# Jittor/InstanceSegmentation-jittor

Measured on AMD Instinct MI355X. Metric: images/sec (Yolact R50-FPN 550x550, bs=8 per GPU, fp32), higher is better.
Workload: dtype f32; 1 GPU; Yolact R50-FPN 550x550 bs=8/GPU random weights: uint8 upload + FastBaseTransform on the device + backbone+FPN+protonet+heads+Detect(fast-NMS)+550x550 mask assembly (BASELINE configs[1]); global_batch=8, parallelism=batch-sharded x1, RCCL all-gather of detections

## Files before the change

### instancesegmentation-jittor_amd/csrc/engine.h

```cpp
#pragma once
#include "rpn_levels.h"
#include <stdarg.h>

#include <functional>
#include <map>
#include <string>
#include <vector>

#include "../../include/isegmi.h"
#include "common.h"

#define TRY(x)               \
    do {                     \
        int _rc = (x);       \
        if (_rc) return _rc; \
    } while (0)

namespace isegmi {

struct Tensor {
    float* d = nullptr;
    int N = 0, H = 0, W = 0, C = 0;
    int dt = 0;
    int64_t numel() const { return (int64_t)N * H * W * C; }
};

struct ConvLayer {
    int Cout = 0, R = 0, S = 0, Cin = 0;
    float* d_w = nullptr;
    bool f16 = false;
    float* d_scale = nullptr;
    float* d_shift = nullptr;
};

struct RawBuf {
    void* d = nullptr;
    int64_t bytes = 0;
    std::vector<int64_t> shape;
    int dtype = 0;
};

struct StageTime {
    std::string name;
    hipEvent_t ev;
};

constexpr float STEP_OVERLAP_DEFAULT = 1.0f;

struct Engine {
    int kind = 0;
    int max_batch = 0, H = 0, W = 0;
    int cur_H = 0, cur_W = 0;
    int anchor_H = -1, anchor_W = -1;
    hipStream_t stream = nullptr;
    hipStream_t side[3] = {nullptr, nullptr, nullptr};
    hipStream_t cur = nullptr;
    hipStream_t tail = nullptr;
    hipEvent_t tail_done = nullptr;
    bool tail_pending = false;
    hipStream_t heads = nullptr;
    hipStream_t hside[3] = {nullptr, nullptr, nullptr};
    hipEvent_t lat_done[2] = {nullptr, nullptr};
    bool lat_pending[2] = {false, false};
    hipEvent_t heads_done = nullptr;
    bool heads_pending = false;
    bool multi_stream = true;
    hipStream_t lane_stream[2] = {nullptr, nullptr};
    hipStream_t lane_side[2][3] = {{nullptr, nullptr, nullptr}, {nullptr, nullptr, nullptr}};
    int lane_state = 0;
    int lane = 0;
    int lane_next = 0;
    int last_lanes = 1;
    bool lane1_busy = false;
    int64_t lane1_forwards = 0;
    std::string lane_tag;
    bool capturing = false;
    std::map<std::string, hipGraphExec_t> graphs;
    std::map<std::string, int> graph_warm;
    int64_t graph_captures = 0, graph_replays = 0, graph_failures = 0;
    hipStream_t copy = nullptr;
    hipEvent_t in_done[2] = {nullptr, nullptr};
    bool in_pending[2] = {false, false};
    struct Upload { const char* dst = nullptr; int64_t bytes = 0; hipEvent_t done = nullptr; unsigned waited = ~0u; };
    unsigned lane_mask() const { return lane_state == 1 ? 3u : 1u; }
    bool consumed(const Upload& u) const { return (u.waited & lane_mask()) == lane_mask(); }
    std::vector<Upload> uploads;
    std::vector<hipEvent_t> step_marks;
    char* pin_ring = nullptr;
    static constexpr int PIN_SLOTS = 32, PIN_SLOT_BYTES = 4096;
    hipEvent_t pin_ev[PIN_SLOTS] = {};
    bool pin_used[PIN_SLOTS] = {};
    int pin_next = 0;
    int hw_slot = 0;
    void* stream_set = nullptr;
    hipEvent_t dl_done[2] = {nullptr, nullptr};
    bool dl_used[2] = {false, false};
    bool fp16 = false;
    std::vector<hipEvent_t> ev_pool;
    size_t ev_next = 0;
    std::map<std::string, ConvLayer> convs;
    std::map<std::string, RawBuf> tensors;
    std::map<std::string, RawBuf> bufs;
    std::map<std::string, float> params;
    bool finalized = false;
    std::vector<int32_t> last_hw;
    const void* last_hw_ptr = nullptr;
    std::vector<float> last_ratios;
    const void* last_ratios_ptr = nullptr;
    int last_N = 0;
    bool timing = false;
    std::vector<StageTime> marks;
    std::vector<std::pair<std::string, float>> last_times;
    bool conv_timing = false;
    std::vector<std::pair<hipEvent_t, hipEvent_t>> conv_evs;
    std::vector<std::pair<std::string, double>> conv_ev_info;
    bool conv_trace = false;
    std::map<std::string, std::pair<double, double>> conv_layers;
    double conv_flops_pending = 0, conv_flops = 0, conv_ms = 0;
    int64_t conv_launches = 0;
    bool op_timing = false;
    struct OpEv { hipEvent_t a, b; const char* label; double bytes; };
    std::vector<OpEv> op_evs;
    struct OpStat { double us = 0, bytes = 0; int64_t launches = 0; };
    std::map<std::string, OpStat> op_stats;

    float param(const std::string& k, float def) const {
        auto it = params.find(k);
        return it == params.end() ? def : it->second;
    }
};

int eng_buf(Engine& e, const std::string& name, int64_t bytes, void** out, int dtype = 0,
            std::vector<int64_t> shape = {});
int eng_act(Engine& e, const std::string& name, int N, int H, int W, int C, Tensor* t, int dt = 0);
int eng_conv(Engine& e, const std::string& layer, const Tensor& in, int stride, int pad, int act, const Tensor* residual,
             const std::string& out_name, Tensor* out, bool out_f32 = false, bool may_split = false);
int eng_graph_run(Engine& e, const std::string& key, const std::function<int()>& body);
void eng_graph_reset(Engine& e);
int eng_tail_end(Engine& e);
int eng_input_consumed(Engine& e);
int eng_wait_upload(Engine& e, const void* d_ptr, int64_t bytes, hipStream_t st);
int eng_stage_small(Engine& e, const void* h_src, size_t bytes, void* d_dst, hipStream_t st);
hipStream_t eng_results_stream(Engine& e);
int eng_bottleneck_f16(Engine& e, const std::string& block, const Tensor& x, bool first, const std::string& out_name, Tensor* out, bool* fused);
int eng_conv_up2x_f16(Engine& e, const std::string& layer, const Tensor& x, const Tensor& coarse, const std::string& out_name, Tensor* out, bool* merged);
struct ConvGroupItem {
    std::string layer;
    Tensor in;
    int stride = 1, pad = 0, act = 0;
    const Tensor* residual = nullptr;
    std::string out_name;
    Tensor* out = nullptr;
    void* dst = nullptr;
    int out_div = 0;
    int64_t out_img_stride = 0, out_pix_stride = 0;
    bool out_f32 = false;
};
int eng_conv_group(Engine& e, std::vector<ConvGroupItem>& items);
int conv2d_group_launch(int n, const isegmi_conv_desc* const* d, const float* const* in, const float* const* w, const float* const* scale,
                        const float* const* shift, const float* const* res, float* const* out, hipStream_t st);
int eng_rpn_head_f16(Engine& e, const std::string& conv, const std::string& headl, const Tensor& x, const std::string& out_name, Tensor* out, bool* fused);
int eng_stem_pool_f16(Engine& e, const std::string& layer, const Tensor& halo, int H, int W, const std::string& out_name, Tensor* out, bool* fused);
int eng_conv_stem_f16(Engine& e, const std::string& layer, const Tensor& halo, int H, int W, const std::string& out_name, Tensor* out);
int eng_conv_into(Engine& e, const std::string& layer, const Tensor& in, int stride, int pad, int act, void* dst, int out_div,
                  int64_t out_img_stride, int64_t out_pix_stride, bool out_f32 = false);
void eng_mark(Engine& e, const char* name);
int eng_fork(Engine& e, int k);
int eng_join(Engine& e, int k);
struct SideScope {
    Engine& e;
    hipStream_t saved;
    SideScope(Engine& e_, int k) : e(e_), saved(e_.cur) { if (e.multi_stream) e.cur = e.side[k]; }
    ~SideScope() { e.cur = saved; }
};

struct OpScope {
    Engine& e;
    hipStream_t st;
    const char* label;
    double bytes;
    hipEvent_t a = nullptr;
    OpScope(Engine& e_, hipStream_t st_, const char* label_, double bytes_) : e(e_), st(st_), label(label_), bytes(bytes_) {
        if (e.op_timing && !e.capturing && hipEventCreate(&a) == hipSuccess) (void)hipEventRecord(a, st);
    }
    ~OpScope() {
        if (!a) return;
        hipEvent_t b = nullptr;
        if (hipEventCreate(&b) == hipSuccess) { (void)hipEventRecord(b, st); e.op_evs.push_back({a, b, label, bytes}); }
        else (void)hipEventDestroy(a);
    }
};

struct ConvScope {
    Engine& e;
    hipEvent_t a = nullptr, b = nullptr;
    explicit ConvScope(Engine& e_) : e(e_) {
        if (!e.conv_timing) return;
        if (hipEventCreate(&a) == hipSuccess && hipEventCreate(&b) == hipSuccess && hipEventRecord(a, e.cur) == hipSuccess) return;
        drop();
    }
    ~ConvScope() { drop(); }
    void drop() {
        if (a) (void)hipEventDestroy(a);
        if (b) (void)hipEventDestroy(b);
        a = b = nullptr;
    }
    void trace(const std::string& layer, const char* suffix, int N, int H, int W, int Cin, int Cout, int R, int stride, int M, bool res) const {
        if (e.conv_trace) fprintf(stderr, "convlaunch\t%s%s\t%d\t%d\t%d\t%d\t%d\t%d\t%d\t%d\t%d\n", layer.c_str(), suffix, N, H, W, Cin, Cout, R, stride, M, res ? 1 : 0);
    }
    __attribute__((format(printf, 3, 4))) void done(double flops, const char* label_fmt, ...) {
        if (!a) return;
        char label[320];
        va_list ap;
        va_start(ap, label_fmt);
        vsnprintf(label, sizeof(label), label_fmt, ap);
        va_end(ap);
        (void)hipEventRecord(b, e.cur);
        e.conv_evs.push_back({a, b});
        e.conv_ev_info.push_back({label, flops});
        e.conv_flops_pending += flops;
        a = b = nullptr;
    }
};

int resnet_stem(Engine& e, const std::string& layer, const float* d_images, int N, int H, int W, Tensor* pool);
struct ResStage {
    std::string layers;
    std::string bufs;
    int blocks = 0;
    int stride = 1;
    bool stride_in_1x1 = false;
    bool full = false;
    std::string stage;
    bool proj_by_name = false;
    hipEvent_t before_out = nullptr;
};
int resnet_stage(Engine& e, const ResStage& s, const Tensor& in, Tensor* out);
bool eng_has_gn(Engine& e, const std::string& layer);
int eng_gn(Engine& e, const std::string& layer, Tensor* x, const Tensor* residual, bool relu);

int yolact_forward(Engine& e, const float* d_images, int N);
int yolact_postprocess(Engine& e, int h, int w, const int32_t* h_image_hw = nullptr);
int maskrcnn_forward(Engine& e, const float* d_images, int N);
int eng_next_event(Engine& e, hipEvent_t* ev);
int maskrcnn_paste(Engine& e, const float* h_ratios_wh, int out_h, int out_w);

int conv2d_launch(const isegmi_conv_desc* d, const float* in, const float* w, const float* scale, const float* shift,
                  const float* res, float* out, hipStream_t st);
int conv2d_f16_launch(const isegmi_conv_desc* d, const void* in, const void* w, const float* scale, const float* shift, const void* res,
                      void* out, int out_f32, hipStream_t st);
int conv2d_f16_up2x_launch(const isegmi_conv_desc* d, const void* in, const void* w, const float* scale, const float* shift, const void* coarse, int Hc, int Wc,
                           void* out, hipStream_t st);
int conv2d_f16_head_launch(const isegmi_conv_desc* d, const void* in, const void* w, const float* scale, const float* shift, const void* w2,
                           const float* scale2, const float* shift2, int cout2, float* out2, bool* fused, hipStream_t st);
bool stem_pool_f16_supported(int Cout);
int stem_pool_f16_launch(int N, int H, int W, const void* halo, const void* w, const float* scale, const float* shift, void* out, int flags, hipStream_t st);
bool bottleneck_f16_supported(int Cin, int Cmid);
bool bottleneck_f16_ds_supported(int Cin, int Cmid);
int bottleneck_f16_launch(const isegmi_bottleneck_desc* d, const void* x, const void* w1, const float* s1, const float* b1, const void* w2,
                          const float* s2, const float* b2, const void* w3, const float* s3, const float* b3, const void* wd, const float* sd,
                          const float* bd, void* out, hipStream_t st);
int pad_c3_to_f16_halo_launch(const float* in, int N, int H, int W, void* out, hipStream_t st);
int avgpool_full_launch(const float* x, int64_t R, int HW, int C, float* out, hipStream_t st);
int resize_bilinear_f16_launch(const void* in, int N, int H, int W, int C, int Ho, int Wo, const void* add, int relu, void* out, hipStream_t st);
int maxpool_to_f16_launch(const void* in, int in_f16, int N, int H, int W, int C, int k, int s, int p, void* out, hipStream_t st);
int nearest2x_add_f16_launch(const void* coarse, int N, int Hc, int Wc, int C, const void* lat, int H, int W, void* out, hipStream_t st);
int roi_align_f16_launch(const void* const* feats, const int* Hs, const int* Ws, const float* scales, int nlevels, const float* rois,
                         const int* counts, int N, int K, int C, int PH, int PW, int g, int k_min, void* out, hipStream_t st,
                         const int* order = nullptr, const void* tab = nullptr, int aligned = 0);
int roi_prep_launch(const float* rois, const int* counts, int N, int K, const int* Hs, const int* Ws, const float* scales, int nlevels, int k_min, int C,
                    int PH, int PW, int esize, int* order, void* tab, hipStream_t st, int aligned = 0);
int mask_logits_select_f16_launch(const void* feat, int R, int HW, int C, const float* w, const float* b, const int* labels, float* out,
                                  hipStream_t st);
int maxpool_launch(const float* in, int N, int H, int W, int C, int k, int s, int p, float* out, hipStream_t st);
int64_t groupnorm_workspace_bytes(int64_t N, int H, int W, int C, int groups);
bool groupnorm_is_slab(int H, int W);
int groupnorm_launch(const float* x, int64_t N, int H, int W, int C, int groups, const float* gamma, const float* beta, float eps, const float* residual,
                     int relu, float* out, void* ws, int64_t ws_bytes, hipStream_t st);
int resize_bilinear_launch(const float* in, int N, int H, int W, int C, int Ho, int Wo, const float* add, int relu, float* out,
                           hipStream_t st);
int nearest2x_add_launch(const float* coarse, int N, int Hc, int Wc, int C, const float* lat, int H, int W, float* out,
                         hipStream_t st);
int maskiou_conv1_launch(const float* lo, int NK, int PH, int PW, const float* w, const float* b, float* out, hipStream_t st);
int maskiou_rescore_launch(const float* feat, int N, int K, int HW, int C, const int* cls, const float* score, const int* count,
                           float* out, hipStream_t st);
int deform_im2col_launch(const float* x, int N, int H, int W, int C, const float* om, int R, int S, int stride, int pad, int dil,
                         float* out, hipStream_t st);
int pad_c3_c4_launch(const float* in, int64_t npix, float* out, hipStream_t st);
int preprocess_u8_launch(const uint8_t* in, int N, int Hin, int Win, float* out, int Hout, int Wout, int Hpad, int Wpad, int64_t out_img_stride,
                         const float* mean3, const float* std3, int swap_rb, hipStream_t st);
int pad_c3_c32_launch(const float* in, int64_t npix, float* out, hipStream_t st);
int topk_launch(const float* keys, int64_t row_stride, int rows, int n, int k, const int* limit, int rows_per_limit,
                float* out_vals, int* out_idx, int* out_cnt, hipStream_t st);
int yolact_detect_launch(const isegmi_yolact_detect_args* a, hipStream_t st);
int yolact_masks_launch(const float* proto, const float* coeffs, const float* boxes, const int* count, int N, int PH, int PW,
                        int mask_dim, int K, int h, int w, float* ws_lo, uint8_t* out_masks, int64_t* out_boxes, hipStream_t st,
                        const int* image_hw = nullptr, int* win = nullptr, bool clear = true, bool dense_lo = false);

}

struct isegmi_engine {
    isegmi::Engine e;
};
```

### instancesegmentation-jittor_amd/csrc/yolact.cpp

```cpp
#include <string.h>

#include "engine.h"

namespace isegmi {

struct LaneScope {
    Engine& e;
    explicit LaneScope(Engine& e_) : e(e_) { set(e.lane); if (e.lane) e.lane_tag = "@1"; }
    ~LaneScope() { set(0); e.lane_tag.clear(); e.cur = e.stream; }
    void set(int l) {
        if (e.lane_stream[l] == nullptr) return;
        e.stream = e.lane_stream[l];
        for (int k = 0; k < 3; ++k) e.side[k] = e.lane_side[l][k];
    }
};

struct HeadsScope {
    Engine& e;
    hipStream_t s, sd[3];
    bool on = false;
    explicit HeadsScope(Engine& e_) : e(e_), s(e_.stream) { for (int k = 0; k < 3; ++k) sd[k] = e.side[k]; }
    void enter(bool wide) { on = true; e.stream = e.heads; for (int k = 0; k < 3; ++k) e.side[k] = wide ? e.hside[k] : e.heads; e.cur = e.heads; }
    ~HeadsScope() { if (on) { e.stream = s; for (int k = 0; k < 3; ++k) e.side[k] = sd[k]; e.cur = s; } }
};
// ... 141 lines not shown
    if (e.multi_stream && e.tail_pending && !e.capturing) HIP_TRY(hipStreamWaitEvent(e.stream, e.tail_done, 0));
    Tensor proto;
    TRY(eng_fork(e, 0));
    TRY(eng_fork(e, 1));
    TRY(eng_fork(e, 2));
    {
        SideScope sc(e, 0);
        Tensor t, u;
        TRY(eng_conv(e, "proto_net.0", P[0], 1, 1, 1, nullptr, "proto.t0", &t));
        TRY(eng_conv(e, "proto_net.2", t, 1, 1, 1, nullptr, "proto.t1", &u));
        TRY(eng_conv(e, "proto_net.4", u, 1, 1, 1, nullptr, "proto.t2", &t));
        TRY(eng_act(e, "proto.up", N, t.H * 2, t.W * 2, t.C, &u, dt));
        if (dt) TRY(resize_bilinear_f16_launch(t.d, N, t.H, t.W, t.C, t.H * 2, t.W * 2, nullptr, 1, u.d, e.cur));
        else TRY(resize_bilinear_launch(t.d, N, t.H, t.W, t.C, t.H * 2, t.W * 2, nullptr, 1, u.d, e.cur));
        TRY(eng_conv(e, "proto_net.8", u, 1, 1, 1, nullptr, "proto.t3", &t));
        TRY(eng_conv(e, "proto_net.10", t, 1, 0, 1, nullptr, "proto", &proto, true));
    }
    if (grp) {
        Tensor uf[5];
        std::vector<ConvGroupItem> gu(5), gh(5);
        for (int l = 0; l < 5; ++l) {
            gu[l].layer = "prediction_layers.0.upfeature.0"; gu[l].in = P[l]; gu[l].pad = 1; gu[l].act = 1; gu[l].out_name = "head.up" + std::to_string(l); gu[l].out = &uf[l];
        }
        TRY(eng_conv_group(e, gu));
        for (int l = 0; l < 5; ++l) {
            gh[l].layer = "prediction_layers.0.head_cat"; gh[l].in = uf[l]; gh[l].pad = 1; gh[l].act = 0;
            gh[l].dst = (float*)headcat + (int64_t)(off[l] / A) * CH; gh[l].out_div = uf[l].H * uf[l].W;
            gh[l].out_img_stride = (int64_t)(Ptot / A) * CH; gh[l].out_pix_stride = CH; gh[l].out_f32 = true;
        }
        TRY(eng_conv_group(e, gh));
    } else {
        { SideScope sc(e, 1); TRY(head_level(1)); TRY(head_level(3)); }
        { SideScope sc(e, 2); TRY(head_level(2)); TRY(head_level(4)); }
        TRY(head_level(0));
    }
    TRY(eng_join(e, 0));
    TRY(eng_join(e, 1));
    TRY(eng_join(e, 2));
    h->A = A; h->Ptot = Ptot; h->CH = CH; h->fused = fused;
    h->loc = loc; h->conf = conf; h->mask = mask; h->headcat = headcat;
    return ISEGMI_OK;
}

static int detect_args(Engine& e, int N, const HeadOut& h, isegmi_yolact_detect_args* out) {
    const int ncls = kNumClasses, md = kMaskDim, A = h.A, Ptot = h.Ptot;
    const int top_k = (int)e.param("nms_top_k", 200), max_det = (int)e.param("max_num_detections", 100);
    const int nc = ncls - 1;
    isegmi_yolact_detect_args& a = *out;
    memset(&a, 0, sizeof(a));
    a.N = N; a.P = Ptot; a.ncls = ncls; a.mask_dim = md; a.top_k = top_k; a.max_det = max_det;
    a.conf_thresh = e.param("nms_conf_thresh", 0.05f);
    a.nms_thresh = e.param("nms_thresh", 0.5f);
    a.second_threshold = (int)e.param("nms_second_threshold", 0) ? 1 : 0;
    if (h.fused) {
        a.d_conf = a.d_loc = a.d_mask = (const float*)h.headcat;
        a.A = A; a.pix_stride = h.CH; a.off_loc = 0; a.off_conf = A * 4; a.off_mask = A * 4 + A * ncls; a.mask_tanh = 1;
    } else {
        a.d_conf = (const float*)h.conf; a.d_loc = (const float*)h.loc; a.d_mask = (const float*)h.mask;
    }
    a.d_priors = (const float*)e.tensors["priors"].d;
    void* p;
    TRY(eng_buf(e, "ws.scoresT", (int64_t)N * nc * Ptot * 4, &p)); a.d_ws_scoresT = (float*)p;
    TRY(eng_buf(e, "boxes_all", (int64_t)N * Ptot * 16, &p, 0, {N, Ptot, 4})); a.d_ws_boxes = (float*)p;
    TRY(eng_buf(e, "ws.counts", (int64_t)2 * N * 4, &p, 1)); a.d_ws_counts = (int32_t*)p;
    TRY(eng_buf(e, "ws.tk_vals", (int64_t)N * nc * top_k * 4, &p)); a.d_ws_tk_vals = (float*)p;
    TRY(eng_buf(e, "ws.tk_idx", (int64_t)N * nc * top_k * 4, &p, 1)); a.d_ws_tk_idx = (int32_t*)p;
    TRY(eng_buf(e, "ws.tk_cnt", (int64_t)N * nc * 4, &p, 1)); a.d_ws_tk_cnt = (int32_t*)p;
    TRY(eng_buf(e, "ws.cand", (int64_t)N * nc * top_k * 4, &p)); a.d_ws_cand = (float*)p;
    TRY(eng_buf(e, "ws.fin_vals", (int64_t)N * max_det * 4, &p)); a.d_ws_fin_vals = (float*)p;
    TRY(eng_buf(e, "ws.fin_idx", (int64_t)N * max_det * 4, &p, 1)); a.d_ws_fin_idx = (int32_t*)p;
    TRY(eng_buf(e, "ws.fin_cnt", (int64_t)N * 4, &p, 1)); a.d_ws_fin_cnt = (int32_t*)p;
    TRY(eng_buf(e, "det.count", (int64_t)N * 4, &p, 1, {N})); a.d_out_count = (int32_t*)p;
    TRY(eng_buf(e, "det.box", (int64_t)N * max_det * 16, &p, 0, {N, max_det, 4})); a.d_out_boxes = (float*)p;
    TRY(eng_buf(e, "det.score", (int64_t)N * max_det * 4, &p, 0, {N, max_det})); a.d_out_scores = (float*)p;
    TRY(eng_buf(e, "det.class", (int64_t)N * max_det * 4, &p, 1, {N, max_det})); a.d_out_classes = (int32_t*)p;
    TRY(eng_buf(e, "det.coeff", (int64_t)N * max_det * md * 4, &p, 0, {N, max_det, md})); a.d_out_coeffs = (float*)p;
    TRY(eng_buf(e, "det.prior", (int64_t)N * max_det * 4, &p, 1, {N, max_det})); a.d_out_prior = (int32_t*)p;
    return ISEGMI_OK;
}

int yolact_forward(Engine& e, const float* d_images, int N) {
    LaneScope lscope(e);
    e.cur = e.stream;
    const bool pipe = e.multi_stream && !e.capturing && !e.timing && !e.conv_timing && e.heads != nullptr &&
                      e.param("graph", 0.0f) == 0.0f && e.param("pipeline_heads", 1.0f) != 0.0f;
    HeadsScope hscope(e);
    eng_mark(e, "start");
    const int dt = e.fp16 ? 1 : 0;
    if (dt && e.convs.count("prediction_layers.0.head_cat") == 0) { set_error("fp16 Yolact needs the fused prediction head"); return ISEGMI_ERR_STATE; }
    Tensor C[3], P[5];
    if (e.param("darknet", 0.0f) != 0.0f) TRY(darknet_backbone(e, d_images, N, C));
    else TRY(resnet_backbone(e, d_images, N, C));
    if (pipe) {
        hipEvent_t ev;
        TRY(eng_next_event(e, &ev));
        HIP_TRY(hipEventRecord(ev, e.stream));
        HIP_TRY(hipStreamWaitEvent(e.heads, ev, 0));
        const float hs = e.param("heads_side_streams", -1.0f);
        hscope.enter(hs < 0.0f ? N <= 2 : hs != 0.0f);
    } else if (e.heads_pending) {
        HIP_TRY(hipStreamWaitEvent(e.stream, e.heads_done, 0));
        e.heads_pending = false;
    }
    const bool grp = !dt && e.param("conv_groups", 1.0f) != 0.0f && e.param("conv_tile", 0) == 0.0f && e.convs.count("prediction_layers.0.head_cat") != 0;
    TRY(yolact_fpn(e, C, N, grp, pipe, P));
    eng_mark(e, "fpn");
    e.lane_tag.clear();
    HeadOut head;
    TRY(proto_and_heads(e, P, N, grp, &head));
    eng_mark(e, "proto+heads");
    isegmi_yolact_detect_args a;
    TRY(detect_args(e, N, head, &a));
    hipStream_t ds = e.stream;
    if (e.multi_stream) {
        hipEvent_t ev;
        TRY(eng_next_event(e, &ev));
        HIP_TRY(hipEventRecord(ev, e.stream));
        HIP_TRY(hipStreamWaitEvent(e.tail, ev, 0));
        ds = e.tail;
    }
    {
        OpScope op(e, ds, "yolact_detect (softmax + decode + per-class top-k + fast-NMS + gather)",
                   (double)N * a.P * ((double)(4 + a.ncls - 1 + a.mask_dim) * 4) + (double)a.P * 16);
        TRY(yolact_detect_launch(&a, ds));
    }
    if (pipe) { HIP_TRY(hipEventRecord(e.heads_done, e.stream)); e.heads_pending = true; }
    TRY(eng_tail_end(e));
    eng_mark(e, "detect");
    return ISEGMI_OK;
}

int yolact_postprocess(Engine& e, int h, int w, const int32_t* h_image_hw) {
    const int N = e.last_N;
    if (N <= 0) { set_error("postprocess before forward"); return ISEGMI_ERR_STATE; }
    const int K = (int)e.param("max_num_detections", 100);
    RawBuf& proto = e.bufs["proto"];
    const int PH = (int)proto.shape[1], PW = (int)proto.shape[2], md = (int)proto.shape[3];
    void *lo, *masks, *ib;
    hipStream_t rs = (e.multi_stream && e.tail_pending) ? e.tail : e.stream;
    int* d_ihw = nullptr;
    if (h_image_hw) {
        for (int i = 0; i < N; ++i)
            if (h_image_hw[2 * i] <= 0 || h_image_hw[2 * i] > h || h_image_hw[2 * i + 1] <= 0 || h_image_hw[2 * i + 1] > w) { set_error("postprocess: image size outside the plane"); return ISEGMI_ERR_ARG; }
        void* q;
        TRY(eng_buf(e, "pp.image_hw", (int64_t)e.max_batch * 8, &q, 1, {N, 2}));
        d_ihw = (int*)q;
        TRY(eng_stage_small(e, h_image_hw, (size_t)N * 8, d_ihw, rs));
    }
    TRY(eng_buf(e, "ws.lo", (int64_t)N * K * PH * PW * 4, &lo));
    TRY(eng_buf(e, "det.masks", (int64_t)N * K * h * w, &masks, 2, {N, K, h, w}));
    TRY(eng_buf(e, "det.box_int", (int64_t)N * K * 4 * 8, &ib, 3, {N, K, 4}));
    void* wq;
    TRY(eng_buf(e, "det.mask_window", (int64_t)e.max_batch * K * 16, &wq, 1, {N, K, 4}));
    {
        const bool whole = e.param("sparse_masks", 0.0f) == 0.0f;
        OpScope op(e, rs, whole ? "yolact_masks (proto @ coeff -> sigmoid -> crop -> upsample -> threshold, whole uint8 planes)" : "yolact_masks (sparse: box windows only)",
                   (double)N * PH * PW * md * 4 + (double)N * K * md * 4 + (whole ? (double)N * K * h * w : 0.0));
        TRY(yolact_masks_launch((const float*)proto.d, (const float*)e.bufs["det.coeff"].d, (const float*)e.bufs["det.box"].d,
                                (const int*)e.bufs["det.count"].d, N, PH, PW, md, K, h, w, (float*)lo, (uint8_t*)masks, (int64_t*)ib,
                                rs, d_ihw, (int*)wq, whole, e.convs.count("maskiou_net.2") != 0));
    }
    if (e.convs.count("maskiou_net.2")) {
        auto w0 = e.tensors.find("maskiou.w0"), b0 = e.tensors.find("maskiou.b0");
        if (w0 == e.tensors.end() || b0 == e.tensors.end()) { set_error("maskiou_net.0 weights missing"); return ISEGMI_ERR_STATE; }
        hipStream_t saved = e.cur;
        e.cur = rs;
        Tensor t, u;
        TRY(eng_act(e, "maskiou.t0", N * K, (PH - 3) / 2 + 1, (PW - 3) / 2 + 1, 32, &t));
        TRY(maskiou_conv1_launch((const float*)lo, N * K, PH, PW, (const float*)w0->second.d, (const float*)b0->second.d, t.d, rs));
        for (int i = 2; i <= 8; i += 2) {
            if (t.H < 3 || t.W < 3) { e.cur = saved; set_error("input too small for the mask-IoU net (five stride-2 3x3 convs)"); return ISEGMI_ERR_ARG; }
            TRY(eng_conv(e, "maskiou_net." + std::to_string(i), t, 2, 0, 1, nullptr, "maskiou.t" + std::to_string(i), &u));
            t = u;
        }
        TRY(eng_conv(e, "maskiou_net.10", t, 1, 0, 1, nullptr, "maskiou.cls", &u));
        void* ms;
        TRY(eng_buf(e, "det.mask_score", (int64_t)N * K * 4, &ms, 0, {N, K}));
        TRY(maskiou_rescore_launch(u.d, N, K, u.H * u.W, u.C, (const int*)e.bufs["det.class"].d, (const float*)e.bufs["det.score"].d,
                                   (const int*)e.bufs["det.count"].d, (float*)ms, rs));
        e.cur = saved;
    }
    if (rs == e.tail) HIP_TRY(hipEventRecord(e.tail_done, e.tail));
    eng_mark(e, "masks");
    return ISEGMI_OK;
}

}
```

### instancesegmentation-jittor_amd/csrc/yolact_detect.hip

```cpp
#include "../../include/isegmi.h"
#include "common.h"
#include "detmath.h"

namespace isegmi {

constexpr int SM_ROWS = 128;

struct HeadLayout {
    int A;
    int64_t pix_stride;
    int off_loc, off_conf, off_mask, mask_tanh;
};
__device__ __forceinline__ const float* head_ptr(const float* base, const HeadLayout& L, int n, int P, int p, int width, int off) {
    if (L.pix_stride == 0) return base + ((int64_t)n * P + p) * width;
    const int pix = p / L.A, a = p - pix * L.A;
    return base + ((int64_t)n * (P / L.A) + pix) * L.pix_stride + off + a * width;
}

constexpr int SM_PARTS = 4;
__global__ __launch_bounds__(SM_ROWS * SM_PARTS) void yolact_softmax_decode_kernel(
    const float* __restrict__ conf, const float* __restrict__ loc, const float* __restrict__ priors, int P, int C,
    float conf_thresh, const HeadLayout L, float* __restrict__ scoresT, float* __restrict__ boxes, int* __restrict__ keep_count) {
    extern __shared__ float sm[];
    constexpr int NT = SM_ROWS * SM_PARTS;
// ... 38 lines not shown
        if (live) {
            const float s = rsum[t];
            for (int c = part; c < C; c += SM_PARTS) { const float pr = dm_div(r[c], s); r[c] = pr; if (c >= 1) fg = pr > fg ? pr : fg; }
        }
        pmax[part * SM_ROWS + t] = fg;
    }
    __syncthreads();
    float fg = pmax[t];
#pragma unroll
    for (int q = 1; q < SM_PARTS; ++q) { const float v = pmax[q * SM_ROWS + t]; fg = v > fg ? v : fg; }
    const bool kept = live && fg > conf_thresh;
    if (live && part == 1) {
        const float* lp = head_ptr(loc, L, n, P, p, 4, L.off_loc);
        const float4 l = make_float4(lp[0], lp[1], lp[2], lp[3]);
        const float4 q = *(const float4*)(priors + (int64_t)p * 4);
        float tx = l.x * 0.1f; tx = tx * q.z;
        float ty = l.y * 0.1f; ty = ty * q.w;
        const float cx = q.x + tx, cy = q.y + ty;
        const float w = q.z * dm_exp(l.z * 0.2f), h = q.w * dm_exp(l.w * 0.2f);
        const float x1 = cx - dm_div(w, 2.0f), y1 = cy - dm_div(h, 2.0f);
        *(float4*)(boxes + ((int64_t)n * P + p) * 4) = make_float4(x1, y1, w + x1, h + y1);
    }
    const int cnt = __syncthreads_count((kept && part == 0) ? 1 : 0);
    if (threadIdx.x == 0 && cnt) atomicAdd(&keep_count[n], cnt);
    if (live) {
        float* dst = scoresT + (int64_t)n * (C - 1) * P + p;
        for (int c = 1 + part; c < C; c += SM_PARTS) dst[(int64_t)(c - 1) * P] = kept ? r[c] : -1.0f;
    }
}

__device__ __forceinline__ float jaccard(const float4 a, const float4 b) {
    const float mx2 = a.z < b.z ? a.z : b.z, mx1 = a.x > b.x ? a.x : b.x;
    const float my2 = a.w < b.w ? a.w : b.w, my1 = a.y > b.y ? a.y : b.y;
    float iw = mx2 - mx1, ih = my2 - my1;
    iw = iw > 0.0f ? iw : 0.0f;
    ih = ih > 0.0f ? ih : 0.0f;
    const float inter = iw * ih;
    const float aa = (a.z - a.x) * (a.w - a.y), ab = (b.z - b.x) * (b.w - b.y);
    const float uni = aa + ab - inter;
    return dm_div(inter, uni);
}

__global__ __launch_bounds__(1024) void yolact_fast_nms_kernel(const float* __restrict__ boxes, const float* __restrict__ tk_vals,
                                                                const int* __restrict__ tk_idx, const int* __restrict__ tk_cnt,
                                                                int P, int nc, int top_k, float thr, int second_threshold, float conf_thresh,
                                                                float* __restrict__ cand, int* __restrict__ kept_count) {
    __shared__ float4 sb[256];
    __shared__ unsigned char okp[4][256];
    const int c = blockIdx.x, n = blockIdx.y;
    const int base = (n * nc + c) * top_k;
    const int cnt = tk_cnt[n * nc + c];
    const int j = threadIdx.x & 255, part = threadIdx.x >> 8;
    if (part == 0 && j < cnt) sb[j] = *(const float4*)(boxes + ((int64_t)n * P + tk_idx[base + j]) * 4);
    __syncthreads();
    bool ok = true;
    if (j < cnt) {
        const float4 bj = sb[j];
        for (int i = part; i < j; i += 4) {
            const float o = jaccard(sb[i], bj);
            if (!(o <= thr)) { ok = false; break; }
        }
    }
    okp[part][j] = ok ? 1 : 0;
    __syncthreads();
    bool keep = part == 0 && j < cnt && okp[0][j] && okp[1][j] && okp[2][j] && okp[3][j];
    if (second_threshold && keep) keep = tk_vals[base + j] > conf_thresh;
    if (part == 0 && j < top_k) cand[base + j] = keep ? tk_vals[base + j] : -1.0f;
    const int k = __syncthreads_count(keep ? 1 : 0);
    if (threadIdx.x == 0 && k) atomicAdd(&kept_count[n], k);
}

__global__ void yolact_gather_kernel(const float* __restrict__ boxes, const float* __restrict__ mask, const int* __restrict__ tk_idx,
                                     const float* __restrict__ fin_vals, const int* __restrict__ fin_idx,
                                     const int* __restrict__ fin_cnt, int P, int nc, int top_k, int mask_dim, int max_det,
                                     const HeadLayout L,
                                     int* __restrict__ out_count, float* __restrict__ out_boxes, float* __restrict__ out_scores,
                                     int* __restrict__ out_classes, float* __restrict__ out_coeffs, int* __restrict__ out_prior) {
    const int n = blockIdx.x;
    const int cnt = fin_cnt[n];
    if (threadIdx.x == 0) out_count[n] = cnt;
    for (int q = threadIdx.x; q < max_det; q += blockDim.x) {
        const int64_t o = (int64_t)n * max_det + q;
        if (q < cnt) {
            const int flat = fin_idx[o];
            const int c = flat / top_k;
            const int prior = tk_idx[(int64_t)n * nc * top_k + flat];
            *(float4*)(out_boxes + o * 4) = *(const float4*)(boxes + ((int64_t)n * P + prior) * 4);
            out_scores[o] = fin_vals[o];
            out_classes[o] = c;
            out_prior[o] = prior;
            const float* mp = head_ptr(mask, L, n, P, prior, mask_dim, L.off_mask);
            for (int k = 0; k < mask_dim; ++k) out_coeffs[o * mask_dim + k] = L.mask_tanh ? dm_tanh(mp[k]) : mp[k];
        } else {
            *(float4*)(out_boxes + o * 4) = make_float4(0.f, 0.f, 0.f, 0.f);
            out_scores[o] = 0.0f;
            out_classes[o] = -1;
            out_prior[o] = -1;
            for (int k = 0; k < mask_dim; ++k) out_coeffs[o * mask_dim + k] = 0.0f;
        }
    }
}

__device__ __forceinline__ void sanitize(float a, float b, int img, float padding, float& o1, float& o2) {
    a = a * (float)img; b = b * (float)img;
    float lo = a < b ? a : b, hi = a > b ? a : b;
    lo = lo - padding; hi = hi + padding;
    lo = lo > 0.0f ? lo : 0.0f;
    hi = hi < (float)img ? hi : (float)img;
    o1 = lo; o2 = hi;
}

constexpr int MD = 32;
constexpr int PROTO_DG = 25;
template <bool DENSE>
__global__ __launch_bounds__(256) void yolact_proto_masks_kernel(const float* __restrict__ proto, const float* __restrict__ coeffs,
                                                                  const float* __restrict__ boxes, const int* __restrict__ count,
                                                                  int PH, int PW, int K, float* __restrict__ lo) {
    extern __shared__ float sm[];
    const int n = blockIdx.y;
    const int d_lo = blockIdx.z * PROTO_DG;
    const int cnt = count[n] < d_lo + PROTO_DG ? count[n] : d_lo + PROTO_DG;
    if (d_lo >= cnt) return;
    float* sc = sm;
    float* sw = sm + K * MD;
    for (int i = d_lo * MD + threadIdx.x; i < cnt * MD; i += 256) sc[i] = coeffs[(int64_t)n * K * MD + i];
    for (int d = d_lo + threadIdx.x; d < cnt; d += 256) {
        const float4 b = *(const float4*)(boxes + ((int64_t)n * K + d) * 4);
        float x1, x2, y1, y2;
        sanitize(b.x, b.z, PW, 1.0f, x1, x2);
        sanitize(b.y, b.w, PH, 1.0f, y1, y2);
        sw[d * 4 + 0] = x1; sw[d * 4 + 1] = x2; sw[d * 4 + 2] = y1; sw[d * 4 + 3] = y2;
    }
    __syncthreads();
    const int pix = blockIdx.x * 256 + threadIdx.x;
    if (pix >= PH * PW) return;
    const int y = pix / PW, x = pix - y * PW;
    float pv[MD];
    const float4* ps = (const float4*)(proto + ((int64_t)n * PH * PW + pix) * MD);
#pragma unroll
    for (int k = 0; k < MD / 4; ++k) { const float4 v = ps[k]; pv[4 * k] = v.x; pv[4 * k + 1] = v.y; pv[4 * k + 2] = v.z; pv[4 * k + 3] = v.w; }
    const float fx = (float)x, fy = (float)y;
    for (int d = d_lo; d < cnt; ++d) {
        const bool inside = fx >= sw[d * 4] && fx < sw[d * 4 + 1] && fy >= sw[d * 4 + 2] && fy < sw[d * 4 + 3];
        if (!DENSE && !inside) continue;
        const float* cf = sc + d * MD;
        float acc = 0.0f;
#pragma unroll
        for (int k = 0; k < MD; ++k) acc = fmaf(pv[k], cf[k], acc);
        const float v = dm_sigmoid(acc);
        lo[(((int64_t)n * K + d) * PH * PW) + pix] = inside ? v : 0.0f;
    }
}

__global__ __launch_bounds__(256) void yolact_upsample_masks_kernel(const float* __restrict__ lo, const float* __restrict__ boxes,
                                                                     const int* __restrict__ count, int PH, int PW, int K, int h, int w,
                                                                     const int* __restrict__ image_hw, uint8_t* __restrict__ out, int* __restrict__ win) {
    const int n = blockIdx.z, d = blockIdx.y;
    if (d >= count[n]) return;
    const int plane_w = w;
    const int64_t plane = (int64_t)h * w;
    if (image_hw) { h = image_hw[2 * n]; w = image_hw[2 * n + 1]; }
    const float4 b = *(const float4*)(boxes + ((int64_t)n * K + d) * 4);
    float x1, x2, y1, y2;
    sanitize(b.x, b.z, PW, 1.0f, x1, x2);
    sanitize(b.y, b.w, PH, 1.0f, y1, y2);
    const float fsx = (float)w / (float)PW, fsy = (float)h / (float)PH;
    int ox0 = (int)floorf((ceilf(x1) - 1.0f + 0.5f) * fsx - 0.5f) - 2, ox1 = (int)ceilf((ceilf(x2) + 0.5f) * fsx - 0.5f) + 2;
    int oy0 = (int)floorf((ceilf(y1) - 1.0f + 0.5f) * fsy - 0.5f) - 2, oy1 = (int)ceilf((ceilf(y2) + 0.5f) * fsy - 0.5f) + 2;
    ox0 = ox0 < 0 ? 0 : ox0; ox1 = ox1 > w ? w : ox1;
    oy0 = oy0 < 0 ? 0 : oy0; oy1 = oy1 > h ? h : oy1;
    const int ww = ox1 - ox0, wh = oy1 - oy0;
    if (win != nullptr && blockIdx.x == 0 && threadIdx.x == 0) { int* wq = win + ((int64_t)n * K + d) * 4; wq[0] = ox0; wq[1] = oy0; wq[2] = ox1; wq[3] = oy1; }
    if (ww <= 0 || wh <= 0) return;
    const int area = ww * wh;
    const float sy = dm_div((float)PH, (float)h), sx = dm_div((float)PW, (float)w);
    const float* m = lo + ((int64_t)n * K + d) * PH * PW;
    uint8_t* o = out + ((int64_t)n * K + d) * plane;
    auto tap = [&](int yy, int xx) -> float {
        const float fx = (float)xx, fy = (float)yy;
        return (fx >= x1 && fx < x2 && fy >= y1 && fy < y2) ? m[yy * PW + xx] : 0.0f;
    };
    for (int i = blockIdx.x * 256 + threadIdx.x; i < area; i += gridDim.x * 256) {
        const int ry = i / ww;
        const int y = oy0 + ry, x = ox0 + (i - ry * ww);
        int y0, yb, x0, xb; float ly0, ly1, lx0, lx1;
        dm_bil_coef_s(y, PH, sy, y0, yb, ly0, ly1);
        dm_bil_coef_s(x, PW, sx, x0, xb, lx0, lx1);
        float top = lx0 * tap(y0, x0); top = fmaf(lx1, tap(y0, xb), top);
        float bot = lx0 * tap(yb, x0); bot = fmaf(lx1, tap(yb, xb), bot);
        float v = ly0 * top; v = fmaf(ly1, bot, v);
        o[y * plane_w + x] = v > 0.5f ? (uint8_t)1 : (uint8_t)0;
    }
}

__global__ void yolact_int_boxes_kernel(const float* __restrict__ boxes, const int* __restrict__ count, int K, int h, int w,
                                        const int* __restrict__ image_hw, int64_t* __restrict__ out) {
    const int n = blockIdx.x;
    if (image_hw) { h = image_hw[2 * n]; w = image_hw[2 * n + 1]; }
    for (int d = threadIdx.x; d < K; d += blockDim.x) {
        int64_t* o = out + ((int64_t)n * K + d) * 4;
        if (d < count[n]) {
            const float4 b = *(const float4*)(boxes + ((int64_t)n * K + d) * 4);
            float x1, x2, y1, y2;
            sanitize(b.x, b.z, w, 0.0f, x1, x2);
            sanitize(b.y, b.w, h, 0.0f, y1, y2);
            o[0] = (int64_t)x1; o[1] = (int64_t)y1; o[2] = (int64_t)x2; o[3] = (int64_t)y2;
        } else { o[0] = o[1] = o[2] = o[3] = 0; }
    }
}

int topk_launch(const float* keys, int64_t row_stride, int rows, int n, int k, const int* limit, int rows_per_limit,
                float* out_vals, int* out_idx, int* out_cnt, hipStream_t st);

int yolact_detect_launch(const isegmi_yolact_detect_args* a, hipStream_t st) {
    ARG_CHECK(a->N > 0 && a->P > 0 && a->ncls >= 2 && a->ncls <= 256, "detect sizes");
    ARG_CHECK(a->top_k > 0 && a->top_k <= 256 && a->max_det > 0 && a->max_det <= 128, "top_k<=256, max_det<=128");
    ARG_CHECK(a->mask_dim > 0, "mask_dim");
    const int nc = a->ncls - 1;
    HIP_TRY(hipMemsetAsync(a->d_ws_counts, 0, sizeof(int) * 2 * (size_t)a->N, st));
    int* keep_count = a->d_ws_counts;
    int* kept2 = a->d_ws_counts + a->N;
    const size_t lds = ((size_t)SM_ROWS * a->ncls + (size_t)(SM_PARTS + 1) * SM_ROWS) * sizeof(float);
    HeadLayout L;
    L.A = a->A > 0 ? a->A : 1; L.pix_stride = a->pix_stride; L.off_loc = a->off_loc; L.off_conf = a->off_conf; L.off_mask = a->off_mask;
    L.mask_tanh = a->mask_tanh;
    ARG_CHECK(a->pix_stride == 0 || (a->A > 0 && a->P % a->A == 0), "fused head layout needs A > 0 and P % A == 0");
    hipLaunchKernelGGL(yolact_softmax_decode_kernel, dim3(cdiv(a->P, SM_ROWS), a->N), dim3(SM_ROWS * SM_PARTS), lds, st, a->d_conf, a->d_loc,
                       a->d_priors, a->P, a->ncls, a->conf_thresh, L, a->d_ws_scoresT, a->d_ws_boxes, keep_count);
    HIP_TRY(hipGetLastError());
    int rc = topk_launch(a->d_ws_scoresT, a->P, a->N * nc, a->P, a->top_k, keep_count, nc, a->d_ws_tk_vals, a->d_ws_tk_idx,
                         a->d_ws_tk_cnt, st);
    if (rc) return rc;
    hipLaunchKernelGGL(yolact_fast_nms_kernel, dim3(nc, a->N), dim3(1024), 0, st, a->d_ws_boxes, a->d_ws_tk_vals, a->d_ws_tk_idx,
                       a->d_ws_tk_cnt, a->P, nc, a->top_k, a->nms_thresh, a->second_threshold, a->conf_thresh, a->d_ws_cand, kept2);
    HIP_TRY(hipGetLastError());
    rc = topk_launch(a->d_ws_cand, (int64_t)nc * a->top_k, a->N, nc * a->top_k, a->max_det, kept2, 1, a->d_ws_fin_vals,
                     a->d_ws_fin_idx, a->d_ws_fin_cnt, st);
    if (rc) return rc;
    hipLaunchKernelGGL(yolact_gather_kernel, dim3(a->N), dim3(128), 0, st, a->d_ws_boxes, a->d_mask, a->d_ws_tk_idx, a->d_ws_fin_vals,
                       a->d_ws_fin_idx, a->d_ws_fin_cnt, a->P, nc, a->top_k, a->mask_dim, a->max_det, L, a->d_out_count,
                       a->d_out_boxes, a->d_out_scores, a->d_out_classes, a->d_out_coeffs, a->d_out_prior);
    HIP_TRY(hipGetLastError());
    return ISEGMI_OK;
}

__global__ __launch_bounds__(256) void maskiou_conv1_kernel(const float* __restrict__ lo, int64_t total, int PH, int PW, int Ho, int Wo,
                                                            const float* __restrict__ w, const float* __restrict__ b,
                                                            float* __restrict__ out) {
    __shared__ float sw[72], sb[8];
    if (threadIdx.x < 72) sw[threadIdx.x] = w[threadIdx.x];
    if (threadIdx.x < 8) sb[threadIdx.x] = b[threadIdx.x];
    __syncthreads();
    for (int64_t t = (int64_t)blockIdx.x * 256 + threadIdx.x; t < total; t += (int64_t)gridDim.x * 256) {
        const int wo = (int)(t % Wo);
        const int64_t q = t / Wo;
        const int ho = (int)(q % Ho);
        const int64_t img = q / Ho;
        const float* src = lo + (img * PH + 2 * ho) * PW + 2 * wo;
        float x[9];
#pragma unroll
        for (int r = 0; r < 3; ++r)
#pragma unroll
            for (int c = 0; c < 3; ++c) x[r * 3 + c] = src[r * PW + c];
        float y[8];
#pragma unroll
        for (int co = 0; co < 8; ++co) {
            float acc = 0.0f;
#pragma unroll
            for (int k = 0; k < 9; ++k) acc = fmaf(x[k], sw[co * 9 + k], acc);
            const float v = fmaf(acc, 1.0f, sb[co]) + 0.0f;
            y[co] = v > 0.0f ? v : 0.0f;
        }
        float4* d = (float4*)(out + t * 32);
        d[0] = make_float4(y[0], y[1], y[2], y[3]);
        d[1] = make_float4(y[4], y[5], y[6], y[7]);
        const float4 z = make_float4(0.f, 0.f, 0.f, 0.f);
#pragma unroll
        for (int k = 2; k < 8; ++k) d[k] = z;
    }
}
__global__ void maskiou_rescore_kernel(const float* __restrict__ feat, int HW, int C, const int* __restrict__ cls,
                                       const float* __restrict__ score, const int* __restrict__ count, int K,
                                       float* __restrict__ out) {
    const int n = blockIdx.x;
    for (int d = threadIdx.x; d < K; d += blockDim.x) {
        float r = 0.0f;
        if (d < count[n]) {
            const float* f = feat + ((int64_t)n * K + d) * HW * C + cls[n * K + d];
            float m = f[0];
            for (int p = 1; p < HW; ++p) { const float v = f[(int64_t)p * C]; m = v > m ? v : m; }
            r = score[n * K + d] * m;
        }
        out[n * K + d] = r;
    }
}
int maskiou_conv1_launch(const float* lo, int NK, int PH, int PW, const float* w, const float* b, float* out, hipStream_t st) {
    ARG_CHECK(PH >= 3 && PW >= 3, "mask-IoU net input smaller than 3x3");
    const int Ho = (PH - 3) / 2 + 1, Wo = (PW - 3) / 2 + 1;
    const int64_t total = (int64_t)NK * Ho * Wo;
    int64_t blocks = cdiv64(total, 256);
    if (blocks > 65536) blocks = 65536;
    hipLaunchKernelGGL(maskiou_conv1_kernel, dim3((unsigned)blocks), dim3(256), 0, st, lo, total, PH, PW, Ho, Wo, w, b, out);
    HIP_TRY(hipGetLastError());
    return ISEGMI_OK;
}
int maskiou_rescore_launch(const float* feat, int N, int K, int HW, int C, const int* cls, const float* score, const int* count,
                           float* out, hipStream_t st) {
    hipLaunchKernelGGL(maskiou_rescore_kernel, dim3(N), dim3(128), 0, st, feat, HW, C, cls, score, count, K, out);
    HIP_TRY(hipGetLastError());
    return ISEGMI_OK;
}

int yolact_masks_launch(const float* proto, const float* coeffs, const float* boxes, const int* count, int N, int PH, int PW,
                        int mask_dim, int K, int h, int w, float* ws_lo, uint8_t* out_masks, int64_t* out_boxes, hipStream_t st,
                        const int* image_hw, int* win, bool clear, bool dense_lo) {
    ARG_CHECK(mask_dim == MD, "mask_dim must be 32");
    ARG_CHECK(N > 0 && K > 0 && K <= 128 && h > 0 && w > 0, "mask sizes");
    const size_t lds = (size_t)K * (MD + 4) * sizeof(float);
    if (dense_lo)
        hipLaunchKernelGGL(yolact_proto_masks_kernel<true>, dim3(cdiv(PH * PW, 256), N, cdiv(K, PROTO_DG)), dim3(256), lds, st, proto, coeffs, boxes, count,
                           PH, PW, K, ws_lo);
    else
        hipLaunchKernelGGL(yolact_proto_masks_kernel<false>, dim3(cdiv(PH * PW, 256), N, cdiv(K, PROTO_DG)), dim3(256), lds, st, proto, coeffs, boxes, count,
                           PH, PW, K, ws_lo);
    HIP_TRY(hipGetLastError());
    ARG_CHECK((int64_t)h * w < (1ll << 31), "h * w must stay below 2^31");
    if (clear) HIP_TRY(hipMemsetAsync(out_masks, 0, (size_t)N * K * h * w, st));
    int chunks = (int)cdiv64((int64_t)h * w, 2048);
    if (chunks > 32) chunks = 32;
    hipLaunchKernelGGL(yolact_upsample_masks_kernel, dim3((unsigned)chunks, (unsigned)K, (unsigned)N), dim3(256), 0, st, ws_lo, boxes, count, PH, PW, K, h, w,
                       image_hw, out_masks, win);
    HIP_TRY(hipGetLastError());
    if (out_boxes) {
        hipLaunchKernelGGL(yolact_int_boxes_kernel, dim3(N), dim3(128), 0, st, boxes, count, K, h, w, image_hw, out_boxes);
        HIP_TRY(hipGetLastError());
    }
    return ISEGMI_OK;
}

}

using namespace isegmi;

extern "C" int isegmi_op_yolact_detect(const isegmi_yolact_detect_args* a, void* stream) {
    ARG_CHECK(a, "null args");
    return yolact_detect_launch(a, (hipStream_t)stream);
}
extern "C" int isegmi_op_yolact_masks(const float* d_proto, const float* d_coeffs, const float* d_boxes, const int* d_count,
                                      int N, int PH, int PW, int mask_dim, int K, int h, int w, float* d_ws_lo,
                                      uint8_t* d_out_masks, int64_t* d_out_boxes, void* stream) {
    return yolact_masks_launch(d_proto, d_coeffs, d_boxes, d_count, N, PH, PW, mask_dim, K, h, w, d_ws_lo, d_out_masks, d_out_boxes,
                               (hipStream_t)stream, nullptr, nullptr, true, false);
}
```

Measured before the change: 1012 img/s.

## Fuse mask-plane zeroing into upsample kernel and skip planes already cleared

Replaces the full memset of the uint8 mask planes with extra zeroing blocks inside the upsample kernel. Those blocks clear only the region outside each detection's box window. Planes beyond the current detection count are cleared only if the previous call wrote them, tracked by a double-buffered per-image count array on the device. This cuts the write traffic of clearing every full 550x550 plane each batch, but it depends on the output buffer persisting unchanged between calls.

```diff
diff --git a/instancesegmentation-jittor_amd/csrc/engine.h b/instancesegmentation-jittor_amd/csrc/engine.h
--- a/instancesegmentation-jittor_amd/csrc/engine.h
+++ b/instancesegmentation-jittor_amd/csrc/engine.h
@@ -108,6 +108,7 @@
     std::vector<float> last_ratios;
     const void* last_ratios_ptr = nullptr;
     int last_N = 0;
+    struct MaskPlanes { const void* ptr = nullptr; int N = 0, K = 0, h = 0, w = 0, parity = 0; bool valid = false; } mask_planes;
     bool timing = false;
     std::vector<StageTime> marks;
     std::vector<std::pair<std::string, float>> last_times;
@@ -295,7 +296,8 @@
 int yolact_detect_launch(const isegmi_yolact_detect_args* a, hipStream_t st);
 int yolact_masks_launch(const float* proto, const float* coeffs, const float* boxes, const int* count, int N, int PH, int PW,
                         int mask_dim, int K, int h, int w, float* ws_lo, uint8_t* out_masks, int64_t* out_boxes, hipStream_t st,
-                        const int* image_hw = nullptr, int* win = nullptr, bool clear = true, bool dense_lo = false);
+                        const int* image_hw = nullptr, int* win = nullptr, bool whole = true, bool dense_lo = false,
+                        const int* prev_count = nullptr, int* prev_out = nullptr);
 
 }
 
diff --git a/instancesegmentation-jittor_amd/csrc/yolact.cpp b/instancesegmentation-jittor_amd/csrc/yolact.cpp
--- a/instancesegmentation-jittor_amd/csrc/yolact.cpp
+++ b/instancesegmentation-jittor_amd/csrc/yolact.cpp
@@ -317,13 +317,21 @@
     TRY(eng_buf(e, "det.box_int", (int64_t)N * K * 4 * 8, &ib, 3, {N, K, 4}));
     void* wq;
     TRY(eng_buf(e, "det.mask_window", (int64_t)e.max_batch * K * 16, &wq, 1, {N, K, 4}));
+    void* pv;
+    TRY(eng_buf(e, "pp.mask_prev", (int64_t)2 * e.max_batch * 4, &pv, 1, {2, e.max_batch}));
     {
         const bool whole = e.param("sparse_masks", 0.0f) == 0.0f;
         OpScope op(e, rs, whole ? "yolact_masks (proto @ coeff -> sigmoid -> crop -> upsample -> threshold, whole uint8 planes)" : "yolact_masks (sparse: box windows only)",
                    (double)N * PH * PW * md * 4 + (double)N * K * md * 4 + (whole ? (double)N * K * h * w : 0.0));
+        Engine::MaskPlanes& mp = e.mask_planes;
+        const bool known = whole && mp.valid && mp.ptr == masks && mp.N == N && mp.K == K && mp.h == h && mp.w == w;
+        int* prev = (int*)pv;
         TRY(yolact_masks_launch((const float*)proto.d, (const float*)e.bufs["det.coeff"].d, (const float*)e.bufs["det.box"].d,
                                 (const int*)e.bufs["det.count"].d, N, PH, PW, md, K, h, w, (float*)lo, (uint8_t*)masks, (int64_t*)ib,
-                                rs, d_ihw, (int*)wq, whole, e.convs.count("maskiou_net.2") != 0));
+                                rs, d_ihw, (int*)wq, whole, e.convs.count("maskiou_net.2") != 0,
+                                known ? prev + mp.parity * e.max_batch : nullptr, whole ? prev + (mp.parity ^ 1) * e.max_batch : nullptr));
+        mp.ptr = masks; mp.N = N; mp.K = K; mp.h = h; mp.w = w; mp.valid = whole;
+        if (whole) mp.parity ^= 1;
     }
     if (e.convs.count("maskiou_net.2")) {
         auto w0 = e.tensors.find("maskiou.w0"), b0 = e.tensors.find("maskiou.b0");
diff --git a/instancesegmentation-jittor_amd/csrc/yolact_detect.hip b/instancesegmentation-jittor_amd/csrc/yolact_detect.hip
--- a/instancesegmentation-jittor_amd/csrc/yolact_detect.hip
+++ b/instancesegmentation-jittor_amd/csrc/yolact_detect.hip
@@ -214,11 +214,35 @@
     }
 }
 
+__device__ __forceinline__ void zero_bytes(uint8_t* __restrict__ p, int64_t a, int64_t b, int t, int nt) {
+    if (a >= b) return;
+    int64_t A = a + (int64_t)((16u - (unsigned)(((uintptr_t)p + (uintptr_t)a) & 15u)) & 15u);
+    A = A < b ? A : b;
+    const int64_t B = A + ((b - A) & ~(int64_t)15);
+    for (int64_t i = a + t; i < A; i += nt) p[i] = 0;
+    uint4* q = (uint4*)(p + A);
+    const int64_t nw = (B - A) >> 4;
+    for (int64_t i = t; i < nw; i += nt) q[i] = make_uint4(0u, 0u, 0u, 0u);
+    for (int64_t i = B + t; i < b; i += nt) p[i] = 0;
+}
+
 __global__ __launch_bounds__(256) void yolact_upsample_masks_kernel(const float* __restrict__ lo, const float* __restrict__ boxes,
                                                                      const int* __restrict__ count, int PH, int PW, int K, int h, int w,
-                                                                     const int* __restrict__ image_hw, uint8_t* __restrict__ out, int* __restrict__ win) {
+                                                                     const int* __restrict__ image_hw, uint8_t* __restrict__ out, int* __restrict__ win,
+                                                                     int chunks, int zb, const int* __restrict__ prev, int* __restrict__ prev_out) {
     const int n = blockIdx.z, d = blockIdx.y;
-    if (d >= count[n]) return;
+    const int cnt = count[n];
+    const bool zrole = (int)blockIdx.x >= chunks;
+    const int z = (int)blockIdx.x - chunks;
+    const int plane_h = h;
+    if (prev_out != nullptr && blockIdx.x == 0 && d == 0 && threadIdx.x == 0) prev_out[n] = cnt;
+    if (d >= cnt) {
+        if (zrole && (prev == nullptr || d < prev[n])) {
+            const int64_t pl = (int64_t)h * w;
+            zero_bytes(out + ((int64_t)n * K + d) * pl, pl * z / zb, pl * (z + 1) / zb, threadIdx.x, 256);
+        }
+        return;
+    }
     const int plane_w = w;
     const int64_t plane = (int64_t)h * w;
     if (image_hw) { h = image_hw[2 * n]; w = image_hw[2 * n + 1]; }
@@ -233,16 +257,31 @@
     oy0 = oy0 < 0 ? 0 : oy0; oy1 = oy1 > h ? h : oy1;
     const int ww = ox1 - ox0, wh = oy1 - oy0;
     if (win != nullptr && blockIdx.x == 0 && threadIdx.x == 0) { int* wq = win + ((int64_t)n * K + d) * 4; wq[0] = ox0; wq[1] = oy0; wq[2] = ox1; wq[3] = oy1; }
+    uint8_t* o = out + ((int64_t)n * K + d) * plane;
+    if (zrole) {
+        const int ra = (int)((int64_t)plane_h * z / zb), rb = (int)((int64_t)plane_h * (z + 1) / zb);
+        if (ww <= 0 || wh <= 0) { zero_bytes(o, (int64_t)ra * plane_w, (int64_t)rb * plane_w, threadIdx.x, 256); return; }
+        const int ta = ra, tb = rb < oy0 ? rb : oy0;
+        if (ta < tb) zero_bytes(o, (int64_t)ta * plane_w, (int64_t)tb * plane_w, threadIdx.x, 256);
+        const int ba = ra > oy1 ? ra : oy1, bb = rb;
+        if (ba < bb) zero_bytes(o, (int64_t)ba * plane_w, (int64_t)bb * plane_w, threadIdx.x, 256);
+        const int ma = ra > oy0 ? ra : oy0, mb = rb < oy1 ? rb : oy1;
+        const int lane = threadIdx.x & 63, wave = threadIdx.x >> 6;
+        for (int y = ma + wave; y < mb; y += 4) {
+            zero_bytes(o, (int64_t)y * plane_w, (int64_t)y * plane_w + ox0, lane, 64);
+            zero_bytes(o, (int64_t)y * plane_w + ox1, (int64_t)(y + 1) * plane_w, lane, 64);
+        }
+        return;
+    }
     if (ww <= 0 || wh <= 0) return;
     const int area = ww * wh;
     const float sy = dm_div((float)PH, (float)h), sx = dm_div((float)PW, (float)w);
     const float* m = lo + ((int64_t)n * K + d) * PH * PW;
-    uint8_t* o = out + ((int64_t)n * K + d) * plane;
     auto tap = [&](int yy, int xx) -> float {
         const float fx = (float)xx, fy = (float)yy;
         return (fx >= x1 && fx < x2 && fy >= y1 && fy < y2) ? m[yy * PW + xx] : 0.0f;
     };
-    for (int i = blockIdx.x * 256 + threadIdx.x; i < area; i += gridDim.x * 256) {
+    for (int i = blockIdx.x * 256 + threadIdx.x; i < area; i += chunks * 256) {
         const int ry = i / ww;
         const int y = oy0 + ry, x = ox0 + (i - ry * ww);
         int y0, yb, x0, xb; float ly0, ly1, lx0, lx1;
@@ -375,7 +414,7 @@
 
 int yolact_masks_launch(const float* proto, const float* coeffs, const float* boxes, const int* count, int N, int PH, int PW,
                         int mask_dim, int K, int h, int w, float* ws_lo, uint8_t* out_masks, int64_t* out_boxes, hipStream_t st,
-                        const int* image_hw, int* win, bool clear, bool dense_lo) {
+                        const int* image_hw, int* win, bool whole, bool dense_lo, const int* prev_count, int* prev_out) {
     ARG_CHECK(mask_dim == MD, "mask_dim must be 32");
     ARG_CHECK(N > 0 && K > 0 && K <= 128 && h > 0 && w > 0, "mask sizes");
     const size_t lds = (size_t)K * (MD + 4) * sizeof(float);
@@ -387,11 +426,13 @@
                            PH, PW, K, ws_lo);
     HIP_TRY(hipGetLastError());
     ARG_CHECK((int64_t)h * w < (1ll << 31), "h * w must stay below 2^31");
-    if (clear) HIP_TRY(hipMemsetAsync(out_masks, 0, (size_t)N * K * h * w, st));
     int chunks = (int)cdiv64((int64_t)h * w, 2048);
     if (chunks > 32) chunks = 32;
-    hipLaunchKernelGGL(yolact_upsample_masks_kernel, dim3((unsigned)chunks, (unsigned)K, (unsigned)N), dim3(256), 0, st, ws_lo, boxes, count, PH, PW, K, h, w,
-                       image_hw, out_masks, win);
+    int zb = 0;
+    if (whole) { zb = (int)cdiv64((int64_t)h * w, 32768); zb = zb > 16 ? 16 : zb; }
+    ARG_CHECK(prev_count == nullptr || prev_count != prev_out, "prev_count and prev_out must be two arrays");
+    hipLaunchKernelGGL(yolact_upsample_masks_kernel, dim3((unsigned)(chunks + zb), (unsigned)K, (unsigned)N), dim3(256), 0, st, ws_lo, boxes, count, PH, PW, K, h, w,
+                       image_hw, out_masks, win, chunks, zb, whole ? prev_count : nullptr, prev_out);
     HIP_TRY(hipGetLastError());
     if (out_boxes) {
         hipLaunchKernelGGL(yolact_int_boxes_kernel, dim3(N), dim3(128), 0, st, boxes, count, K, h, w, image_hw, out_boxes);
@@ -412,5 +453,5 @@
                                       int N, int PH, int PW, int mask_dim, int K, int h, int w, float* d_ws_lo,
                                       uint8_t* d_out_masks, int64_t* d_out_boxes, void* stream) {
     return yolact_masks_launch(d_proto, d_coeffs, d_boxes, d_count, N, PH, PW, mask_dim, K, h, w, d_ws_lo, d_out_masks, d_out_boxes,
-                               (hipStream_t)stream, nullptr, nullptr, true, false);
-}
+                               (hipStream_t)stream, nullptr, nullptr, true, false, nullptr, nullptr);
+}
```

Measured after the change: 1016 img/s (median of 6 runs). No clear change (+0.4%).
